# PN-CourseWork/02689-AdvancedNumericalAlgorithmP3

Hardware: AMD Instinct MI355X
Metric: steady-state time-steps/sec at N=256 Re=1000 (higher is better)
Workload: dtype f64; 1 GPU; solver=spectral (SG) N=256 Re=1000 fp64, full solve() iteration (dt, 4 RK stages + BCs, change/residual norms, E/Z/P), fluid from rest; N=256, trials_per_gpu=1, parallelism=1 independent trial(s), one per GPU

## Files before the change

02689-advancednumericalalgorithmp3_amd/csrc/ldc_kernels.hip:

```cpp

#include <hip/hip_runtime.h>
#include <stdint.h>
#include <stdlib.h>
#include <string.h>
#include <mutex>
#include <new>
#include <type_traits>
#include <vector>

#include "ldc_hip.h"

namespace {

typedef double v4d __attribute__((ext_vector_type(4)));

#define MFMA_F64(a, b, c) __builtin_amdgcn_mfma_f64_16x16x4f64((a), (b), (c), 0, 0, 0)

#ifdef LDC_TIMING
#define LDC_ABL(x, bits) ((x).ablate & (bits))
#else
#define LDC_ABL(x, bits) 0
#endif

constexpr int kWaves = 4;
// ... 175 lines not shown
  const int jj = loc / pr, i = loc - jj * pr;
  I = pI * pr + i;
  J = pJ * pc + (I + jj) % pc;
}

struct FinalArgs {
  int nblk4, nblkZ, nblkP;
  int with_diag, warmup, nan_guard, rec_cap;
  int do_critical;
  double cfl, beta2, nu, hx, hy, lid, tol;
  const double *part4, *partZ0, *partP0;
  long long stride;
  double* scal;
  int* ctrl;
  double* rec;
};

__device__ __forceinline__ double dt_lambda_x(double umax, const FinalArgs& a) {
  const double um = fmax(umax, a.lid);
  return (um + sqrt(nm_madd(um, um, a.beta2))) / a.hx + a.nu / (a.hx * a.hx);
}
__device__ __forceinline__ double dt_lambda_y(double vmax, const FinalArgs& a) {
  const double vm = fmax(vmax, 1e-10);
  return (vm + sqrt(nm_madd(vm, vm, a.beta2))) / a.hy + a.nu / (a.hy * a.hy);
}
__device__ __forceinline__ double next_dt(double umax, double vmax, const FinalArgs& a) {
  return a.cfl / (dt_lambda_x(umax, a) + dt_lambda_y(vmax, a));
}

struct TrialState {
  int done, iter, step, flushed, pdone, drows;
  int abort;
  unsigned arrive;
  double dt, umax, vmax;
  double dtp;
};

struct StageArgs {
  int M, LD, T, tail;
  int Mx, My;
  double nu, beta2, alpha;
  const double *Dx, *D2x, *Dy, *D2y, *IxF, *GxF;
  const double *Uin, *UinT, *Vin, *VinT;
  const double *U0, *V0, *P0;
  const double *U0T, *V0T;
  const double *T1T, *T2T;
  double *PX, *PY;
  double *Uout, *UoutT, *Vout, *VoutT, *Pout;
  const double *ulid, *wx, *wy;
  const double *DxL, *D2xL, *DyL, *D2yL;
  double *W, *WT;
  double *partZ0, *partP0;
  long long stride;
  const double* scal;
  int* ctrl;
  double* partials;
#ifdef LDC_TIMING
  int ablate;
#endif
  double* dump[11];
  int NB;
  const double *DxK, *D2xK, *DyK, *D2yK, *IxFK, *GxFK;
  const double *UinK, *UinTK, *VinK, *VinTK, *T1TK, *T2TK;
  double *UoutK, *UoutTK, *VoutK, *VoutTK, *PoutK, *WK, *WTK;
  int wt;
  int rm_out;
// ... 2340 lines not shown
```

02689-advancednumericalalgorithmp3_amd/csrc/ldc_wide_kernel.inc:

```

constexpr int kWT = 16;
constexpr int kWTmin = 6;
constexpr int kWD2 = 6;
constexpr int kWD = 4;

struct WArgs {
  int M, LD, NB, T;
  int tail;
  int Mx, My;
  int with_diag;
  double nu, beta2;
  const double *DxK, *D2xK, *DyK, *D2yK, *GxFK, *GyFK;
  const double *ulid, *wx, *wy;
  double *U, *UT, *V, *VT, *P;
  double *UK[3], *UTK[3], *VK[3], *VTK[3], *PK[3];
  double *PTK[3];
  double *WK, *WTK;
  const double *IxF, *IyF;
  const double *Dx, *D2x, *Dy, *D2y, *GxF, *GyF;
  const double *DxL, *D2xL, *DyL, *D2yL;
  double* wedge;
  double* jobs;
  double* ring;
  double* rvec;
// ... 54 lines not shown
  const v2d_t hi = *reinterpret_cast<const v2d_t*>(f + 128 + 2 * lane);
  return (v4d){lo[0], lo[1], hi[0], hi[1]};
}

__device__ __forceinline__ bool wwait_flags(unsigned* flags, unsigned phase, int T, int I, int J, bool all, int lane) {
  const int nwg = T * T;
  int wg[4] = {-1, -1, -1, -1};
  if (all) {
#pragma unroll
    for (int k = 0; k < 4; ++k) wg[k] = (lane + 64 * k < nwg) ? lane + 64 * k : -1;
  } else if (lane < 2 * T) {
    wg[0] = lane < T ? I * T + lane : (lane - T) * T + J;
  }
  unsigned long long t0 = 0;
  for (unsigned spins = 0;; ++spins) {
    unsigned v[4];
#pragma unroll
    for (int k = 0; k < 4; ++k)
      v[k] = ((k == 0 || all) && wg[k] >= 0) ? __hip_atomic_load((LDC_GLOBAL unsigned*)flags + 32 * wg[k], __ATOMIC_RELAXED, __HIP_MEMORY_SCOPE_AGENT) : phase;
    const bool behind = (v[0] < phase) || (v[1] < phase) || (v[2] < phase) || (v[3] < phase);
    if (__builtin_amdgcn_ballot_w64(behind) == 0ull) return true;
    if ((spins & 63u) == 63u) {
      const unsigned long long t = __builtin_amdgcn_s_memrealtime();
      if (t0 == 0) t0 = t;
      else if (t - t0 > kSpinLimitTicks) return false;
    }
  }
}
__device__ __forceinline__ void wgive_up(WArgsC& a, TrialState* S) {
  S->abort = 1;
  __hip_atomic_store((LDC_GLOBAL unsigned*)a.giveup, 1u, __ATOMIC_RELAXED, __HIP_MEMORY_SCOPE_AGENT);
}

__device__ __forceinline__ bool wbar(WArgsC& a, unsigned& phaseA, int T, int bx, int I, int J, int tid, TrialState* S, bool all,
                                     double* stp = nullptr) {
  asm volatile("s_waitcnt vmcnt(0)" ::: "memory");
  WSTAMP(7);
  __syncthreads();
  WSTAMP(8);
  ++phaseA;
  if (tid < 64) {
    if (tid == 0) __hip_atomic_store((LDC_GLOBAL unsigned*)a.flags + 32 * bx, phaseA, __ATOMIC_RELAXED, __HIP_MEMORY_SCOPE_AGENT);
    if (!wwait_flags(a.flags, phaseA, T, I, J, all, tid) && tid == 0) wgive_up(a, S);
    WSTAMP(9);
  }
  __syncthreads();
  WSTAMP(10);
  return S->abort == 0;
}

__device__ __forceinline__ v4d wld4(const double* base, size_t i) {
  const __amdgpu_buffer_rsrc_t r = raw_rsrc(base);
  const int off = (int)(i * sizeof(double));
  const v2d_t lo = __builtin_bit_cast(v2d_t, __builtin_amdgcn_raw_buffer_load_b128(r, off, 0, 16));
  const v2d_t hi = __builtin_bit_cast(v2d_t, __builtin_amdgcn_raw_buffer_load_b128(r, off + 16, 0, 16));
  return (v4d){lo[0], lo[1], hi[0], hi[1]};
}
__device__ __forceinline__ int wrows_padded(int nwg) { return (nwg + 3) & ~3; }

template <bool CONST_A>
__device__ __forceinline__ void wchain2(v4d& r0, v4d& r1, const double* p0, const double* p1, const double* pan, int NB,
                                        int prow, int T, int lane) {
  constexpr int D = kWD2;
  v4d f[D];
#pragma unroll
  for (int d = 0; d < D; ++d) {
    f[d] = ldpk_t<true>(pan, NB, prow, d, lane);
    __builtin_amdgcn_sched_barrier(0);
  }
  v4d c0[2], c1[2];
#pragma unroll
  for (int h = 0; h < 2; ++h) { c0[h] = (v4d){0.0, 0.0, 0.0, 0.0}; c1[h] = (v4d){0.0, 0.0, 0.0, 0.0}; }
  auto mm = [&](const v4d& x, int g) {
    const v4d k0 = wfrag_lds(p0 + g * 256, lane), k1 = wfrag_lds(p1 + g * 256, lane);
#pragma unroll
    for (int s = 0; s < 4; ++s) {
      if (CONST_A) { c0[s & 1] = MFMA_F64(k0[s], x[s], c0[s & 1]); c1[s & 1] = MFMA_F64(k1[s], x[s], c1[s & 1]); }
      else         { c0[s & 1] = MFMA_F64(x[s], k0[s], c0[s & 1]); c1[s & 1] = MFMA_F64(x[s], k1[s], c1[s & 1]); }
    }
  };
  int g = 0;
// ... 189 lines not shown
};
constexpr int kWJobDoubles = 16 * 16;
constexpr double kWJobTag = 7.25e22 + 1977.0;
enum { WJ_UE = 0, WJ_VE, WJ_CD0, WJ_CD1, WJ_CD2, WJ_CD3, WJ_PGS, WJ_PGR, WJ_OMEGA, WJ_WQ, WJ_OPL, WJ_CE0, WJ_CE1, WJ_CE2, WJ_CE3, WJ_UNI };
__device__ __forceinline__ int wjob_id(int kind, int blk, int T) { return kind == 0 ? blk : kind == 1 ? T + blk : 2 * T; }
__device__ __forceinline__ void wjob_load(WArgsC& a, WJob& jb, int T, int lane) {
  const double* base = a.jobs + (size_t)wjob_id(jb.kind, jb.blk, T) * kWJobDoubles;
  const int r = wopaque(lane) & 15;
  jb.ue = xld(base, WJ_UE * 16 + r); jb.ve = xld(base, WJ_VE * 16 + r);
  jb.cd[0] = xld(base, WJ_CD0 * 16 + r); jb.cd[1] = xld(base, WJ_CD1 * 16 + r);
  jb.cd[2] = xld(base, WJ_CD2 * 16 + r); jb.cd[3] = xld(base, WJ_CD3 * 16 + r);
  jb.ce[0] = xld(base, WJ_CE0 * 16 + r); jb.ce[1] = xld(base, WJ_CE1 * 16 + r);
  jb.ce[2] = xld(base, WJ_CE2 * 16 + r); jb.ce[3] = xld(base, WJ_CE3 * 16 + r);
  jb.pgs = xld(base, WJ_PGS * 16 + r); jb.pgr = xld(base, WJ_PGR * 16 + r);
  jb.omega = xld(base, WJ_OMEGA * 16 + r); jb.wq = xld(base, WJ_WQ * 16 + r); jb.opl = xld(base, WJ_OPL * 16 + r);
  jb.am1 = xld(base, WJ_UNI * 16 + 0); jb.am2 = xld(base, WJ_UNI * 16 + 1); jb.wc = xld(base, WJ_UNI * 16 + 2);
}
__device__ __forceinline__ void wjob_store(WArgsC& a, const WJob& jb, int T, int lane_, bool all) {
  const int lane = wopaque(lane_);
  double* base = a.jobs + (size_t)wjob_id(jb.kind, jb.blk, T) * kWJobDoubles;
  if (lane < 16) {
    wst1(base + WJ_PGS * 16 + lane, jb.pgs); wst1(base + WJ_PGR * 16 + lane, jb.pgr); wst1(base + WJ_OMEGA * 16 + lane, jb.omega);
    if (all) {
      wst1(base + WJ_UE * 16 + lane, jb.ue); wst1(base + WJ_VE * 16 + lane, jb.ve);
      wst1(base + WJ_CD0 * 16 + lane, jb.cd[0]); wst1(base + WJ_CD1 * 16 + lane, jb.cd[1]);
      wst1(base + WJ_CD2 * 16 + lane, jb.cd[2]); wst1(base + WJ_CD3 * 16 + lane, jb.cd[3]);
      wst1(base + WJ_CE0 * 16 + lane, jb.ce[0]); wst1(base + WJ_CE1 * 16 + lane, jb.ce[1]);
      wst1(base + WJ_CE2 * 16 + lane, jb.ce[2]); wst1(base + WJ_CE3 * 16 + lane, jb.ce[3]);
      wst1(base + WJ_WQ * 16 + lane, jb.wq); wst1(base + WJ_OPL * 16 + lane, jb.opl);
      if (lane == 0) { wst1(base + WJ_UNI * 16 + 0, jb.am1); wst1(base + WJ_UNI * 16 + 1, jb.am2); wst1(base + WJ_UNI * 16 + 2, jb.wc); }
    }
  }
}
enum { WR_JOBLINE = 64, WR_EXTRA = 96, WR_CGX = 97, WR_CGY = 98, WR_CPX = 99, WR_CPY = 100, WR_JOBRING2 = 104 };

struct WEdgeLoads { double ra[4], rb[4]; v4d f0[4], f1[4]; };
template <int MODE, bool DIAGV>
__device__ __forceinline__ void wedge_issue(WEdgeLoads& w, WArgsC& a, int kind, int blk, const XStageIo io, int T, int w4, int lane_) {
  const int lane = wopaque(lane_);
  const int NB = a.NB;
  const size_t rowm = (size_t)(a.M - 1) * a.LD;
  const double *pan0, *pan1, *rA, *rB;
  if (MODE == 1) {
    pan0 = kind == 0 ? a.VTK[io.in] : a.UK[io.in]; pan1 = kind == 0 ? a.PTK[io.pin] : a.PK[io.pin];
    rA = (kind == 0 ? a.Dx : a.Dy) + rowm; rB = (kind == 0 ? a.GxF : a.GyF) + rowm;
  } else if (MODE == 3) {
    pan0 = kind == 0 ? a.WTK : a.WK; pan1 = pan0;
    rA = (kind == 0 ? a.Dx : a.Dy) + rowm; rB = rA;
  } else {
    pan0 = kind == 0 ? a.UTK[io.in] : a.UK[io.in]; pan1 = kind == 0 ? a.VTK[io.in] : a.VK[io.in];
    rA = (kind == 0 ? a.Dx : a.Dy) + rowm; rB = (kind == 0 ? a.D2x : a.D2y) + rowm;
  }
  constexpr bool use0 = !(MODE == 1 && !DIAGV), use1 = MODE != 3;
#pragma unroll
  for (int m = 0; m < 4; ++m) {
    const int g = w4 + 4 * m, gc = g < T ? g : T - 1;
    const int ko = 16 * gc + 4 * (lane >> 4) + (lane & 3);
    w.ra[m] = *(const LDC_GLOBAL double*)(rA + ko);
    w.rb[m] = use1 ? *(const LDC_GLOBAL double*)(rB + ko) : w.ra[m];
    if (g >= T) { w.ra[m] = 0.0; w.rb[m] = 0.0; }
  }
#pragma unroll
  for (int m = 0; m < 4; ++m) {
    const int g = w4 + 4 * m, gc = g < T ? g : T - 1;
    w.f0[m] = use0 ? ldpk_t<true>(pan0, NB, blk, gc, lane) : (v4d){0.0, 0.0, 0.0, 0.0};
    w.f1[m] = use1 ? ldpk_t<true>(pan1, NB, blk, gc, lane) : w.f0[m];
// ... 151 lines not shown
    G[m] = ldpk(kind == 0 ? a.GxFK : a.GyFK, NB, kind == 0 ? I : J, g, lane);
  }
  for (int m0 = 0; m0 < nblk; m0 += 4) {
    const int m = m0 + (lane >> 4), r = lane & 15;
    const int B = half + 2 * (m < nblk ? m : 0);
    double t[kWT];
#pragma unroll
    for (int L = 0; L < kWT; ++L) {
      const int Lc = L < T ? L : T - 1;
      const size_t o = (size_t)(kind == 0 ? B * T + Lc : Lc * T + B) * 64 + (kind == 0 ? 0 : 32) + c * 16 + r;
      t[L] = xld(a.ring, o);
    }
    double s = 0.0;
#pragma unroll
    for (int L = 0; L < kWT; ++L) s += (L < T) ? t[L] : 0.0;
    if (m < nblk) vec[16 * B + r] = s;
  }
  asm volatile("s_waitcnt lgkmcnt(0)" ::: "memory");
  double s = 0.0;
#pragma unroll
  for (int m = 0; m < (kWT + 1) / 2; ++m) {
    if (m < nblk) {
      const int g = half + 2 * m;
      const v4d av = *reinterpret_cast<const v4d*>(vec + 16 * g + 4 * (lane >> 4));
      s = nm_madd(G[m][0], av[0], s); s = nm_madd(G[m][1], av[1], s);
      s = nm_madd(G[m][2], av[2], s); s = nm_madd(G[m][3], av[3], s);
    }
  }
  s = quad_sum(s);
  if (lane < 16) lds[Ld.RNG + (kind * 2 + half) * 16 + lane] = s;
}

struct WFoldState { bool crit, flush; double umax, vmax; };
__device__ __forceinline__ WFoldState wfold_dt(WArgsC& a, TrialState* S, int T, int I, int J, int lane, unsigned phaseA,
                                               v4d (&fx)[PS_N + 2], double* stp) {
  WFoldState f = {false, false, 0.0, 0.0};
  if (!wwait_flags(a.flags, phaseA, T, I, J, true, lane)) {
    if (lane == 0) wgive_up(a, S);
    return f;
  }
  WSTAMP(1);
  __builtin_amdgcn_s_setprio(3);
  FinalArgs fin;
  __builtin_memcpy(&fin, &a.fin, sizeof(FinalArgs));
  f.crit = fin.do_critical && !S->done && (S->step > S->iter);
  f.flush = fin.with_diag && (S->flushed < S->iter) && (S->pdone >= S->iter);
  const int nwg = T * T, nwp = wrows_padded(nwg), r0 = 4 * lane;
  const bool in = r0 < nwp;
#pragma unroll
  for (int q = 0; q < PS_N + 2; ++q) fx[q] = (v4d){0.0, 0.0, 0.0, 0.0};
  if (f.crit && in) {
    fx[PS_UMAX] = wld4(a.part4, (size_t)PS_UMAX * nwp + r0);
    fx[PS_VMAX] = wld4(a.part4, (size_t)PS_VMAX * nwp + r0);
#pragma unroll
    for (int q = 0; q < PS_NSUM; ++q) fx[q] = wld4(a.part4, (size_t)q * nwp + r0);
  }
  if (f.flush && in) {
    const size_t off = (size_t)((S->iter - 1) & 1) * a.stride + r0;
    fx[PS_N] = wld4(a.partZ0, off);
    fx[PS_N + 1] = wld4(a.partP0, off);
  }
  if (f.crit) {
    auto top = [&](const v4d& x) {
      const double e0 = (r0 < nwg) ? x[0] : 0.0, e1 = (r0 + 1 < nwg) ? x[1] : 0.0;
      const double e2 = (r0 + 2 < nwg) ? x[2] : 0.0, e3 = (r0 + 3 < nwg) ? x[3] : 0.0;
      return wave_top(fmax(fmax(e0, e1), fmax(e2, e3)));
    };
    f.umax = top(fx[PS_UMAX]); f.vmax = top(fx[PS_VMAX]);
  }
  WSTAMP(9);
  return f;
}
__device__ __forceinline__ void wfold_step(WArgsC& a, TrialState* S, const WFoldState& f, int lane) {
  if (f.crit) {
    FinalArgs fin;
    __builtin_memcpy(&fin, &a.fin, sizeof(FinalArgs));
    const double xr = lane == 0 ? dt_lambda_x(f.umax, fin) : lane == 1 ? dt_lambda_y(f.vmax, fin) : 0.0;
    const double lxy = lane_value(xr, 0) + lane_value(xr, 1);
    const double dt_new = fin.cfl / lxy;
    if (lane == 0) { S->dtp = S->dt; S->dt = dt_new; }
  }
  __builtin_amdgcn_s_setprio(0);
}
__device__ __forceinline__ void wfold_record(WArgsC& a, const WLds& Ld, double* lds, TrialState* S, int T, int lane, bool writer,
                                             const WFoldState f, const v4d (&fx)[PS_N + 2], double* stp) {
  if (!f.crit && !f.flush) return;
  FinalArgs fin;
  __builtin_memcpy(&fin, &a.fin, sizeof(FinalArgs));
  const int nwg = T * T, r0 = 4 * lane;
  double* tot = lds + Ld.TOT;
#pragma unroll
  for (int q = 0; q < PS_N + 2; ++q) {
    const double e0 = (r0 < nwg) ? fx[q][0] : 0.0, e1 = (r0 + 1 < nwg) ? fx[q][1] : 0.0;
    const double e2 = (r0 + 2 < nwg) ? fx[q][2] : 0.0, e3 = (r0 + 3 < nwg) ? fx[q][3] : 0.0;
    const bool is_max = (q == PS_UMAX || q == PS_VMAX);
    const double s = is_max ? fmax(fmax(e0, e1), fmax(e2, e3)) : ((e0 + e1) + (e2 + e3));
    const double t = is_max ? wave_top(s) : wave_total(s);
    if (lane == 0) tot[q] = t;
  }
  asm volatile("s_waitcnt lgkmcnt(0)" ::: "memory");
  WSTAMP(11);
  const double dt_cur = f.crit ? S->dtp : S->dt;
  const FinOut o = fin_decide_wave(fin, tot, lane, f.crit, f.flush, S->iter, S->flushed, dt_cur, writer);
  if (lane == 0) {
// ... 55 lines not shown
    const double* pan = wv == 0 ? a.UTK[io.in] : wv == 1 ? a.VTK[io.in] : wv == 2 ? a.UK[io.in] : a.VK[io.in];
    const double* p0 = ops + (xrole ? 0 : 2) * T * 256;
    v4d c0, c1;
    if (xrole) wchain2<true>(c0, c1, p0, p0 + T * 256, pan, NB, J, T, lane);
    else wchain2<false>(c0, c1, p0, p0 + T * 256, pan, NB, I, T, lane);
    WSTAMP(1);
    wput(lds, Ld, wv == 0 ? XR_UX : wv == 1 ? XR_VX : wv == 2 ? XR_UY : XR_VY, c0, lane);
    wput(lds, Ld, wv == 0 ? XR_UXX : wv == 1 ? XR_VXX : wv == 2 ? XR_UYY : XR_VYY, c1, lane);
  } else {
    if (PUBZ && wv == 7 && lane == 0) {
      const double* r = rsum;
      const double x = (((r[0] + r[1]) + (r[2] + r[3])) + ((r[4] + r[5]) + (r[6] + r[7]))) +
                       (((r[8] + r[9]) + (r[10] + r[11])) + ((r[12] + r[13]) + (r[14] + r[15])));
      const int step0 = S->step;
      wst1(a.partZ0 + (size_t)((step0 > 0 ? step0 - 1 : 0) & 1) * a.stride + wopaque_s(bx), TAIL ? x + r[16] : x);
    }
    if (GPV) {
      constexpr bool THREE = !(SP && K == 3);
      const int c1 = THREE ? (2 * T + 1) / 3 : T;
      if (wv == 4) wput(lds, Ld, XR_PX, wchain1<false, true>(nullptr, a.GxFK, I, a.PTK[io.pin], J, NB, c1, lane), lane);
      else if (wv == 5) wput(lds, Ld, XR_PY, wchain1<false, false>(nullptr, a.GyFK, J, a.PK[io.pin], I, NB, c1, lane), lane);
      else if (THREE && wv == 6) {
        wput(lds, Ld, XR_WX, wchain1<false, true>(nullptr, a.GxFK, I, a.PTK[io.pin], J, NB, T - c1, lane, c1), lane);
        wput(lds, Ld, XR_WY, wchain1<false, false>(nullptr, a.GyFK, J, a.PK[io.pin], I, NB, T - c1, lane, c1), lane);
      }
    }
    if (AGRADW) {
      const int h0 = (T + 1) / 2, g0 = wv < 6 ? 0 : h0, ng = wv < 6 ? h0 : T - h0;
      if ((wv & 1) == 0) wput(lds, Ld, wv == 4 ? XR_PX : XR_WX, wchain1<true, true>(ops, nullptr, 0, a.WTK, J, NB, ng, lane, g0), lane);
      else wput(lds, Ld, wv == 5 ? XR_PY : XR_WY, wchain1<true, false>(ops + 2 * T * 256, nullptr, 0, a.WK, I, NB, ng, lane, g0), lane);
    }
    if (RRED && wv == 7 && I == J) wring_reduce(a, T, I, lane);
    if (K == 0 && wv == 7 && fold) {
      fs = wfold_dt(a, S, T, I, J, lane, phaseA, fx, stp);
      wfold_step(a, S, fs, lane);
    }
    if (TAIL && LAST && job) {
      const size_t rowm = (size_t)(a.M - 1) * a.LD;
      const int q0 = (wv - 4) * T / 4, q1 = (wv - 3) * T / 4;
      if (DIAGV && jb.kind < 2) wvec_issue(jvh, a.wedge, jb.kind == 0 ? 0 : (size_t)16 * kWT, q0, q1 - q0, lane);
      if (wv >= 6) wjob_load(a, jb, T, lane);
      if (jb.kind < 2) wedge_issue<4, DIAGV>(jw, a, jb.kind, jb.blk, io, T, wv - 4, lane);
      if (DIAGV && jb.kind == 2 && wv == 7) {
        const double* jbase = a.jobs + (size_t)wjob_id(2, 0, T) * kWJobDoubles;
        const int l4 = 4 * wopaque(lane), n4 = 16 * T;
        jw.ra[0] = xld(jbase, WJ_UNI * 16 + 0); jw.ra[1] = xld(jbase, WJ_UNI * 16 + 1); jw.ra[2] = xld(jbase, WJ_UNI * 16 + 2);
        const bool in = l4 < n4;
        const int lc = in ? l4 : 0;
        jw.f0[0] = *(const LDC_GLOBAL v4d*)(a.Dx + rowm + lc); jw.f0[1] = wld4(a.wedge, (size_t)16 * kWT + lc);
        jw.f0[2] = *(const LDC_GLOBAL v4d*)(a.Dy + rowm + lc); jw.f0[3] = wld4(a.wedge, (size_t)lc);
        if (!in) { jw.f0[0] = (v4d){0.0, 0.0, 0.0, 0.0}; jw.f0[2] = jw.f0[0]; }
      }
      WSTAMP(1);
    }
    if (TAIL && K == 1 && wv == 6 && job) wjob_load(a, jb, T, lane);
    if (RING3 && wv >= 6) {
      if (!wwait_flags(a.flags, phaseA, T, I, J, true, lane)) {
        if (lane == 0) wgive_up(a, S);
      } else {
        if (J == 0 || J == jLast) wring(a, Ld, lds, T, I, J, lane, wv - 6, 0, J == 0 ? 0 : 1);
        if (I == 0 || I == iLast) wring(a, Ld, lds, T, I, J, lane, wv - 6, 1, I == 0 ? 0 : 1);
      }
    }
  }
  WSTAMP(2);
  __syncthreads();
  WSTAMP(3);
  if (S->abort != 0) return false;
  double v[PS_N], ev[PS_N];
#pragma unroll
  for (int q = 0; q < PS_N; ++q) ev[q] = 0.0;
  if (TAIL && K == 1 && wv == 6 && job) { wedge_finish<1, DIAGV>(a, Ld, lds, jb, lane, ev); wjob_store(a, jb, T, lane, false); }
  if (TAIL && LAST && job && wv >= 4) {
    if (jb.kind < 2) wedge_dots<4, DIAGV>(jw, Ld, lds, wv - 4, lane);
    if (DIAGV && jb.kind < 2) {
      const int q0 = (wv - 4) * T / 4, q1 = (wv - 3) * T / 4;
      wvec_finish(jvh, jb.kind == 0 ? ops + 2 * T * 256 : ops, nullptr, 0, NB, q0, q1 - q0, lane, lds + Ld.AXY + 320 + 16 * (wv - 4));
    }
    if (DIAGV && jb.kind == 2 && wv == 7) {
      double sx = 0.0, sy = 0.0;
#pragma unroll
      for (int e = 0; e < 4; ++e) { sx = nm_madd(jw.f0[0][e], jw.f0[1][e], sx); sy = nm_madd(jw.f0[2][e], jw.f0[3][e], sy); }
      const double gxc = wave_total(sx) + jw.ra[0] * jw.ra[2], gyc = wave_total(sy) + jw.ra[1] * jw.ra[2];
      if (lane == 0) { rng[WR_CGX] = gxc; rng[WR_CGY] = gyc; }
    }
  }
  if (tid < 256) {
    auto C = [&](int slot) { return lds[Ld.RES + (slot * 4 + wv) * 64 + lane]; };
    double ux = C(XR_UX), vx = C(XR_VX), uy = C(XR_UY), vy = C(XR_VY);
    double lu = C(XR_UXX) + C(XR_UYY), lv = C(XR_VXX) + C(XR_VYY);
    if (TAIL) { ux += tn.cux; vx += tn.cvx; uy += tn.cuy; vy += tn.cvy; lu += tn.clu; lv += tn.clv; }
    const int blkIJ = I * NB + J, blkJI = J * NB + I;
    double dsum = 0.0;
    if (GPV) {
      constexpr bool THREE = !(SP && K == 3);
      n.px = n.valid ? (THREE ? C(XR_PX) + C(XR_WX) : C(XR_PX)) : 0.0;
      n.py = n.valid ? (THREE ? C(XR_PY) + C(XR_WY) : C(XR_PY)) : 0.0;
    }
    if (RINGE) {
      if (n.rc >= 0) n.px = rng[n.ti];
      if (n.rr >= 0) n.py = rng[32 + n.tj];
    }
    if (RING3) {
      if (n.rc >= 0) n.px = rng[n.ti] + rng[16 + n.ti];
      if (n.rr >= 0) n.py = rng[32 + n.tj] + rng[48 + n.tj];
    }
    if (DIAGE == 1) {
      const double w = n.valid ? (vx - uy) : 0.0;
      wst(a.WK, blkIJ, n.oU, w);
      wst(a.WTK, blkJI, n.oT, w);
      dsum = n.valid ? n.wq * w * w : 0.0;
    }
    if (DIAGE == 2) {
      double gx = C(XR_PX) + C(XR_WX), gy = C(XR_PY) + C(XR_WY);
      if (TAIL) { gx = nm_madd(tn.dxl, wre, gx); gy = nm_madd(wce, tn.dyl, gy); }
      dsum = n.valid ? n.wq * nm_sq2(gx, gy) : 0.0;
    }
    const double Ru = nm_momentum(n.uc, n.vc, ux, uy, n.px, a.nu, lu);
// ... 6 lines not shown
    else if (n.wall) { un = 0.0; vn = 0.0; }
    wst(a.UK[io.out], blkIJ, n.oU, un);
    wst(a.UTK[io.out], blkJI, n.oT, un);
    wst(a.VK[io.out], blkIJ, n.oU, vn);
    wst(a.VTK[io.out], blkJI, n.oT, vn);
    double pn = 0.0;
    if (has_p) {
      pn = n.interior ? nm_madd(adt, Rp, n.p0) : 0.0;
      wst(a.PK[io.pout], blkIJ, n.oU, pn);
      wst(a.PTK[io.pout], blkJI, n.oT, pn);
      if (RPROD) wring_partials(a, Ld, n, lds, pn, bx, lane, wv);
    }
    if (LAST) {
      const double du = un - n.u0, dv = vn - n.v0;
      v[PS_DU2] = n.valid ? du * du : 0.0;
      v[PS_DV2] = n.valid ? dv * dv : 0.0;
      v[PS_U02] = n.valid ? n.u0 * n.u0 : 0.0;
      v[PS_V02] = n.valid ? n.v0 * n.v0 : 0.0;
      v[PS_RU2] = n.valid ? Ru * Ru : 0.0;
      v[PS_RV2] = n.valid ? Rv * Rv : 0.0;
      v[PS_RP2] = n.interior ? Rp * Rp : 0.0;
      v[PS_E] = n.valid ? n.wq * nm_sq2(un, vn) : 0.0;
      v[PS_UMAX] = fabs(un);
      v[PS_VMAX] = fabs(vn);
      n.u0 = un; n.v0 = vn; n.p0 = pn;
    }
    if (DIAGE != 0) {
      const double r = row16_sum(dsum);
      if ((lane & 15) == 0) rsum[n.ti] = r;
    }
    n.uc = un; n.vc = vn;
  }
  WSTAMP(4);
  if (LAST || RPROD) {
    __syncthreads();
    WSTAMP(5);
    if (RPROD) wring_partials_finish(a, Ld, lds, bx, tid);
    if (LAST) {
      constexpr int RS = TAIL ? 272 : 256;
      double* red = lds + Ld.RES;
      if (tid < 256) {
#pragma unroll
        for (int q = 0; q < PS_N; ++q) red[q * RS + tid] = v[q];
      }
      if (TAIL && wv == 7 && job) wedge_finish<5, DIAGV>(a, Ld, lds, jb, lane, ev);
      if (TAIL && wv == 6) {
        if (job) { wedge_finish<3, DIAGV>(a, Ld, lds, jb, lane, ev); wedge_finish<4, DIAGV>(a, Ld, lds, jb, lane, ev); }
        if (lane < 16) {
#pragma unroll
          for (int q = 0; q < PS_N; ++q) red[q * RS + 256 + lane] = ev[q];
        }
      }
      __syncthreads();
      const int nwp = wrows_padded(nwg);
      {
        const double* r = red + wv * RS + lane;
        double y = ((r[0] + r[64]) + r[128]) + r[192];
        if (TAIL) y += (lane < 16) ? r[256] : 0.0;
        const double x = wave_sum(y);
        if (lane == 0) wst1(a.part4 + (size_t)wv * nwp + wopaque_s(bx), x);
      }
      if (wv < 2) {
        const double* r = red + (PS_NSUM + wv) * RS + lane;
        double y = fmax(fmax(r[0], r[64]), fmax(r[128], r[192]));
        if (TAIL) y = fmax(y, (lane < 16) ? r[256] : 0.0);
        const double x = wave_max(y);
        if (lane == 0) wst1(a.part4 + (size_t)(PS_NSUM + wv) * nwp + wopaque_s(bx), x);
      }
      if (DIAGV && tid == 64 * 3) {
        const double* r = rsum;
        const double x = (((r[0] + r[1]) + (r[2] + r[3])) + ((r[4] + r[5]) + (r[6] + r[7]))) +
                         (((r[8] + r[9]) + (r[10] + r[11])) + ((r[12] + r[13]) + (r[14] + r[15])));
        const int step0 = S->step;
        wst1(a.partP0 + (size_t)((step0 > 0 ? step0 - 1 : 0) & 1) * a.stride + wopaque_s(bx), TAIL ? x + r[16] : x);
        S->pdone = step0; S->drows = nwg;
      }
      if (tid == 0) S->step = S->step + 1;
    }
  }
  WSTAMP(6);
  asm volatile("s_waitcnt vmcnt(0)" ::: "memory");
  WSTAMP(7);
  ++phaseA;
  if (lane == 0) __hip_atomic_fetch_add(&S->arrive, 1u, __ATOMIC_RELAXED, __HIP_MEMORY_SCOPE_WORKGROUP);
  if (wv == 0) {
    const unsigned want = 8u * (phaseA - 1u);
    while (__hip_atomic_load(&S->arrive, __ATOMIC_RELAXED, __HIP_MEMORY_SCOPE_WORKGROUP) < want) __builtin_amdgcn_s_sleep(1);
    WSTAMP(8);
    if (tid == 0) __hip_atomic_store((LDC_GLOBAL unsigned*)a.flags + 32 * bx, phaseA, __ATOMIC_RELAXED, __HIP_MEMORY_SCOPE_AGENT);
    if (!wwait_flags(a.flags, phaseA, T, I, J, false, tid) && tid == 0) wgive_up(a, S);
    WSTAMP(9);
  } else if (wv >= 4) {
    if (K == 0 && wv == 7 && fold) wfold_record(a, Ld, lds, S, T, lane, bx == 0, fs, fx, stp);
    if (TAIL && K == 0 && job && jb.kind < 2 && wv < 7) {
      wedge_stream<1, DIAGV>(a, Ld, lds, jb.kind, jb.blk, io, T, wv - 4, lane);
      if (wv == 6) wedge_stream<1, DIAGV>(a, Ld, lds, jb.kind, jb.blk, io, T, 3, lane);
    }
    if (WLINES) {
      if (wv == 4 && (J == 0 || J == jLast)) wring_line(a, T, I, lane, 0, J == 0 ? 0 : 1, rng);
      if (wv == 5 && (I == 0 || I == iLast)) wring_line(a, T, J, lane, 1, I == 0 ? 0 : 1, rng + 32);
      if (job) {
        const size_t rowm = (size_t)(a.M - 1) * a.LD;
        if (DIAGV && jb.kind < 2) wedge_stream<3, DIAGV>(a, Ld, lds, jb.kind, jb.blk, io, T, wv - 4, lane);
        if (wv >= 6 && jb.kind < 2) {
          const int h0 = (T + 1) / 2, g0 = wv == 6 ? 0 : h0, ng = wv == 6 ? h0 : T - h0;
          const int lk = jb.kind == 0 ? 1 : 0;
          WVecHalf vh;
          wvec_issue(vh, a.rvec, (size_t)(2 * lk + 1) * 16 * T, g0, ng, lane);
          wvec_finish(vh, nullptr, lk == 0 ? a.GxFK : a.GyFK, jb.blk, NB, g0, ng, lane,
                      wv == 6 ? rng + (jb.kind == 0 ? 48 : 16) : rng + WR_JOBRING2);
          if (wv == 7 && jb.blk == 0) {
            const double e = jb.kind == 0 ? wvv(a.GxF + rowm, a.rvec, 0, 16 * T, lane)
                                          : wvv(a.GyF + rowm, a.rvec, (size_t)2 * 16 * T, 16 * T, lane);
            if (lane == 0) rng[WR_EXTRA] = e;
          }
        } else if (wv == 6 && jb.kind == 2) {
          const double pxc = wvv(a.GxF + rowm, a.rvec, (size_t)16 * T, 16 * T, lane);
          const double pyc = wvv(a.GyF + rowm, a.rvec, (size_t)3 * 16 * T, 16 * T, lane);
          if (lane == 0) { rng[WR_CPX] = pxc; rng[WR_CPY] = pyc; }
        }
      }
    }
  }
  __syncthreads();
  WSTAMP(10);
  return S->abort == 0;
}

template <bool SP, bool DIAGV, bool TAIL>
__global__ __launch_bounds__(kStageThreads, 2) void wide_kernel(const WLaunch L) {
  static_assert(!(SP && DIAGV), "the smoother carries no diagnostics");
  static_assert(!(SP && TAIL), "the tail layout is built for SG");
  extern __shared__ __attribute__((aligned(16))) double lds[];
  __shared__ TrialState S;
  const int tid = threadIdx.x, lane = tid & 63;
  const int wv = __builtin_amdgcn_readfirstlane(tid >> 6);
  WArgsC& a0 = L.trials ? *(WArgsC*)(uintptr_t)L.trials
                        : *(WArgsC*)((kernarg_ptr)__builtin_amdgcn_kernarg_segment_ptr() + __builtin_offsetof(WLaunch, one));
  const int T = a0.T, nwg = T * T;
  const int trial = (int)blockIdx.x / nwg, bx = (int)blockIdx.x % nwg;
  WArgsC& a = L.trials ? *(WArgsC*)(uintptr_t)(L.trials + trial) : a0;
  const WLds Ld = wlds_of(T);
  const int NB = a.NB, M = a.M, LD = a.LD;
  const int I = bx / T, J = bx % T;
  if (a.fin.ctrl[LDC_CTRL_DONE] != 0) return;
  if (tid == 0) {
    S.done = a.fin.ctrl[LDC_CTRL_DONE]; S.iter = a.fin.ctrl[LDC_CTRL_ITER]; S.step = a.fin.ctrl[LDC_CTRL_STEP];
    S.flushed = a.fin.ctrl[LDC_CTRL_FLUSHED]; S.pdone = a.fin.ctrl[LDC_CTRL_PDONE]; S.drows = a.fin.ctrl[LDC_CTRL_DROWS];
    S.dt = a.fin.scal[LDC_SCAL_DT]; S.umax = a.fin.scal[LDC_SCAL_UMAX]; S.vmax = a.fin.scal[LDC_SCAL_VMAX];
    S.abort = 0; S.arrive = 0u; S.dtp = 0.0;
  }
  for (int q = tid; q < 4 * T * 256; q += kStageThreads) {
    const int p = q / (T * 256), r = q - p * (T * 256), g = r >> 8, e = r & 255;
    const double* src = p == 0 ? a.DxK : p == 1 ? a.D2xK : p == 2 ? a.DyK : a.D2yK;
    const int row = p < 2 ? I : J;
    lds[Ld.OPS + (p * T + g) * 256 + ((e & 3) >> 1) * 128 + (e >> 2) * 2 + (e & 1)] = src[((size_t)(row * NB + g) << 8) + e];
  }
  XNode n;
  n.ti = 4 * (wv & 3) + (lane >> 4); n.tj = lane & 15;
  n.i = 16 * I + n.ti; n.j = 16 * J + n.tj;
  n.oU = xpk(n.ti, n.tj); n.oT = xpk(n.tj, n.ti);
  const int Mx = a.Mx, My = a.My;
  n.valid = (n.i < Mx) && (n.j < My);
  n.interior = (n.i >= 1) && (n.i <= Mx - 2) && (n.j >= 1) && (n.j <= My - 2);
  n.lid = n.valid && (n.j == My - 1);
  n.wall = n.valid && (n.i == 0 || n.i == Mx - 1 || n.j == 0);
  n.rc = !n.valid ? -1 : n.j == 0 ? 0 : n.j == My - 1 ? 1 : -1;
  n.rr = !n.valid ? -1 : n.i == 0 ? 0 : n.i == Mx - 1 ? 1 : -1;
  n.u0 = n.v0 = n.p0 = n.px = n.py = n.lidv = n.wq = 0.0;
  const size_t ij = (size_t)n.i * LD + n.j;
  if (tid < 64) {
    const int c = (tid >> 4) & 1, e = tid & 15;
    const size_t row = c ? (size_t)((tid < 32 ? My : Mx) - 1) * LD : 0;
    lds[Ld.EYX + tid] = (tid < 32) ? a.IyF[row + 16 * J + e] : a.IxF[row + 16 * I + e];
  }
  if (tid < 256) {
    n.u0 = a.U[ij]; n.v0 = a.V[ij]; n.p0 = a.P[ij];
    n.lidv = a.ulid[n.i];
    n.wq = a.wx[n.i] * a.wy[n.j];
    wst(a.UK[0], I * NB + J, n.oU, n.u0); wst(a.UTK[0], J * NB + I, n.oT, n.u0);
    wst(a.VK[0], I * NB + J, n.oU, n.v0); wst(a.VTK[0], J * NB + I, n.oT, n.v0);
    wst(a.PK[0], I * NB + J, n.oU, n.p0);
    wst(a.PTK[0], J * NB + I, n.oT, n.p0);
// ... 25 lines not shown
        WJob jb;
        wjob_init(a, jb, T, I, J, lane);
        wjob_store(a, jb, T, lane, true);
        if (lane == 0) wst1(jbase + WJ_UNI * 16 + 3, kWJobTag);
      }
    }
    if (tid < 16) lds[Ld.RSUM + 16 + tid] = 0.0;
  }
  unsigned phaseA = 0;
  bool alive = wbar(a, phaseA, T, bx, I, J, tid, &S, true);
  bool pending = false;
  for (int it = 0; alive && it < L.n_iters; ++it) {
    if (S.done != 0) break;
#ifdef LDC_TIMING
    const bool stamp = a.stamps != nullptr && it == L.n_iters - 1;
#else
    const bool stamp = false;
#endif
    alive = wstage<SP, DIAGV, TAIL, 0>(a, Ld, n, tn, jkind, jblk, lds, &S, phaseA, T, bx, I, J, pending, stamp);
    if (!alive) break;
    pending = false;
    if (S.done != 0) break;
    alive = wstage<SP, DIAGV, TAIL, 1>(a, Ld, n, tn, jkind, jblk, lds, &S, phaseA, T, bx, I, J, false, stamp);
    if (!alive) break;
    alive = wstage<SP, DIAGV, TAIL, 2>(a, Ld, n, tn, jkind, jblk, lds, &S, phaseA, T, bx, I, J, false, stamp);
    if (!alive) break;
    alive = wstage<SP, DIAGV, TAIL, 3>(a, Ld, n, tn, jkind, jblk, lds, &S, phaseA, T, bx, I, J, false, stamp);
    pending = true;
  }
  if (!alive) return;
  if (pending) {
    if (wv == 7) {
      v4d fx[PS_N + 2];
      const WFoldState fs = wfold_dt(a, &S, T, I, J, lane, phaseA, fx, nullptr);
      wfold_step(a, &S, fs, lane);
      wfold_record(a, Ld, lds, &S, T, lane, bx == 0, fs, fx, nullptr);
    }
    __syncthreads();
    if (S.abort != 0) return;
  }
  double* tu = lds + Ld.RES;
  double* tv = tu + 16 * 17;
  if (tid < 256) {
    a.U[ij] = n.u0; a.V[ij] = n.v0; a.P[ij] = n.p0;
    tu[n.ti * 17 + n.tj] = n.u0; tv[n.ti * 17 + n.tj] = n.v0;
  }
  __syncthreads();
  if (tid < 256) {
    const int tr = tid >> 4, tc = tid & 15;
    const size_t ot = (size_t)(16 * J + tr) * LD + 16 * I + tc;
    a.UT[ot] = tu[tc * 17 + tr];
    a.VT[ot] = tv[tc * 17 + tr];
  }
  if (bx == 0 && tid == 0) {
    a.fin.ctrl[LDC_CTRL_DONE] = S.done; a.fin.ctrl[LDC_CTRL_ITER] = S.iter; a.fin.ctrl[LDC_CTRL_STEP] = S.step;
    a.fin.ctrl[LDC_CTRL_FLUSHED] = S.flushed; a.fin.ctrl[LDC_CTRL_PDONE] = S.pdone; a.fin.ctrl[LDC_CTRL_DROWS] = S.drows;
    a.fin.ctrl[LDC_CTRL_LIVE] = 0;
    a.fin.scal[LDC_SCAL_DT] = S.dt; a.fin.scal[LDC_SCAL_UMAX] = S.umax; a.fin.scal[LDC_SCAL_VMAX] = S.vmax;
  }
}
```

Baseline: 28370 steps/s.

## Publish per-block velocity maxima in flag words to shorten dt critical path

Each workgroup now publishes its u/v maxima, tagged with parity sign bits, directly in its flag cache line. The dt fold can then read all maxima from the flags without waiting for the full partial-sum reduction. The final stage's workgroup barrier is split into per-wave arrive counters (P, D, E, S), so the maxima publish and inter-block flag release happen before the ten partial-sum reductions finish. A separate sums flag gates the later partial loads. This shortens the serial dt dependency between RK iterations, at the cost of more intricate sync logic, extra counters and possible ordering bugs.

```diff
diff --git a/02689-advancednumericalalgorithmp3_amd/csrc/ldc_kernels.hip b/02689-advancednumericalalgorithmp3_amd/csrc/ldc_kernels.hip
--- a/02689-advancednumericalalgorithmp3_amd/csrc/ldc_kernels.hip
+++ b/02689-advancednumericalalgorithmp3_amd/csrc/ldc_kernels.hip
@@ -231,6 +231,7 @@
   int done, iter, step, flushed, pdone, drows;
   int abort;
   unsigned arrive;
+  unsigned arriveP, arriveD, arriveE, arriveS;
   double dt, umax, vmax;
   double dtp;
 };
diff --git a/02689-advancednumericalalgorithmp3_amd/csrc/ldc_wide_kernel.inc b/02689-advancednumericalalgorithmp3_amd/csrc/ldc_wide_kernel.inc
--- a/02689-advancednumericalalgorithmp3_amd/csrc/ldc_wide_kernel.inc
+++ b/02689-advancednumericalalgorithmp3_amd/csrc/ldc_wide_kernel.inc
@@ -110,6 +110,71 @@
   __hip_atomic_store((LDC_GLOBAL unsigned*)a.giveup, 1u, __ATOMIC_RELAXED, __HIP_MEMORY_SCOPE_AGENT);
 }
 
+constexpr int kWFlagSums = 2;
+constexpr int kWFlagMaxBytes = 16;
+constexpr unsigned long long kWSignBit = 1ull << 63;
+__host__ __device__ inline unsigned long long wmax_encode(double x, unsigned sign) {
+  return (__builtin_bit_cast(unsigned long long, x) & ~kWSignBit) | (sign ? kWSignBit : 0ull);
+}
+__host__ __device__ inline double wmax_decode(unsigned long long w) { return __builtin_bit_cast(double, w & ~kWSignBit); }
+__host__ __device__ inline bool wmax_pair_valid(unsigned long long u, unsigned long long v, unsigned parity) {
+  return (unsigned)(u >> 63) == (parity & 1u) && (unsigned)(v >> 63) == ((parity & 1u) ^ 1u);
+}
+__device__ __forceinline__ unsigned witers_of(unsigned phaseA) { return (phaseA - 1u) >> 2; }
+
+__device__ __forceinline__ void wpublish_maxima(unsigned* flags, int bx, double umax, double vmax, unsigned parity) {
+  LDC_GLOBAL unsigned long long* w = (LDC_GLOBAL unsigned long long*)(flags + 32 * bx) + kWFlagMaxBytes / 8;
+  __hip_atomic_store(w, wmax_encode(umax, parity & 1u), __ATOMIC_RELAXED, __HIP_MEMORY_SCOPE_AGENT);
+  __hip_atomic_store(w + 1, wmax_encode(vmax, (parity & 1u) ^ 1u), __ATOMIC_RELAXED, __HIP_MEMORY_SCOPE_AGENT);
+}
+__device__ __forceinline__ bool wwait_maxima(unsigned* flags, unsigned parity, int nwg, int lane, double& umax, double& vmax) {
+  const __amdgpu_buffer_rsrc_t rs = raw_rsrc((const double*)flags);
+  const int r0 = 4 * lane;
+  unsigned long long t0 = 0;
+  for (unsigned spins = 0;; ++spins) {
+    double u[4], v[4];
+    bool behind = false;
+    asm volatile("" ::: "memory");
+#pragma unroll
+    for (int k = 0; k < 4; ++k) {
+      u[k] = 0.0; v[k] = 0.0;
+      if (r0 + k < nwg) {
+        typedef unsigned long long v2u64 __attribute__((ext_vector_type(2)));
+        const v2u64 w = __builtin_bit_cast(v2u64, __builtin_amdgcn_raw_buffer_load_b128(rs, 128 * (r0 + k) + kWFlagMaxBytes, 0, 16));
+        behind = behind || !wmax_pair_valid(w[0], w[1], parity);
+        u[k] = wmax_decode(w[0]); v[k] = wmax_decode(w[1]);
+      }
+    }
+    if (__builtin_amdgcn_ballot_w64(behind) == 0ull) {
+      umax = fmax(fmax(u[0], u[1]), fmax(u[2], u[3]));
+      vmax = fmax(fmax(v[0], v[1]), fmax(v[2], v[3]));
+      return true;
+    }
+    if ((spins & 63u) == 63u) {
+      const unsigned long long t = __builtin_amdgcn_s_memrealtime();
+      if (t0 == 0) t0 = t;
+      else if (t - t0 > kSpinLimitTicks) return false;
+    }
+  }
+}
+__device__ __forceinline__ bool wwait_sums(unsigned* flags, unsigned count, int nwg, int lane) {
+  const int r0 = 4 * lane;
+  unsigned long long t0 = 0;
+  for (unsigned spins = 0;; ++spins) {
+    bool behind = false;
+#pragma unroll
+    for (int k = 0; k < 4; ++k)
+      if (r0 + k < nwg)
+        behind = behind || __hip_atomic_load((LDC_GLOBAL unsigned*)flags + 32 * (r0 + k) + kWFlagSums, __ATOMIC_RELAXED, __HIP_MEMORY_SCOPE_AGENT) < count;
+    if (__builtin_amdgcn_ballot_w64(behind) == 0ull) return true;
+    if ((spins & 63u) == 63u) {
+      const unsigned long long t = __builtin_amdgcn_s_memrealtime();
+      if (t0 == 0) t0 = t;
+      else if (t - t0 > kSpinLimitTicks) return false;
+    }
+  }
+}
+
 __device__ __forceinline__ bool wbar(WArgsC& a, unsigned& phaseA, int T, int bx, int I, int J, int tid, TrialState* S, bool all,
                                      double* stp = nullptr) {
   asm volatile("s_waitcnt vmcnt(0)" ::: "memory");
@@ -125,6 +190,15 @@
   __syncthreads();
   WSTAMP(10);
   return S->abort == 0;
+}
+
+__device__ __forceinline__ void warrive(unsigned* c, int lane) {
+  asm volatile("s_waitcnt lgkmcnt(0)" ::: "memory");
+  if (lane == 0) __hip_atomic_fetch_add(c, 1u, __ATOMIC_RELAXED, __HIP_MEMORY_SCOPE_WORKGROUP);
+}
+__device__ __forceinline__ void wawait(unsigned* c, unsigned want) {
+  while (__hip_atomic_load(c, __ATOMIC_RELAXED, __HIP_MEMORY_SCOPE_WORKGROUP) < want) __builtin_amdgcn_s_sleep(1);
+  asm volatile("" ::: "memory");
 }
 
 __device__ __forceinline__ v4d wld4(const double* base, size_t i) {
@@ -380,6 +454,7 @@
     }
   }
 }
+enum { WRS_JOBSUM = 16, WRS_WAVEMAX = 20, WRS_JOBMAX = 28 };
 enum { WR_JOBLINE = 64, WR_EXTRA = 96, WR_CGX = 97, WR_CGY = 98, WR_CPX = 99, WR_CPY = 100, WR_JOBRING2 = 104 };
 
 struct WEdgeLoads { double ra[4], rb[4]; v4d f0[4], f1[4]; };
@@ -597,23 +672,39 @@
 }
 
 struct WFoldState { bool crit, flush; double umax, vmax; };
-__device__ __forceinline__ WFoldState wfold_dt(WArgsC& a, TrialState* S, int T, int I, int J, int lane, unsigned phaseA,
-                                               v4d (&fx)[PS_N + 2], double* stp) {
+__device__ __forceinline__ WFoldState wfold_dt(WArgsC& a, TrialState* S, int T, int lane, unsigned phaseA, double* stp) {
   WFoldState f = {false, false, 0.0, 0.0};
-  if (!wwait_flags(a.flags, phaseA, T, I, J, true, lane)) {
-    if (lane == 0) wgive_up(a, S);
-    return f;
-  }
-  WSTAMP(1);
-  __builtin_amdgcn_s_setprio(3);
   FinalArgs fin;
   __builtin_memcpy(&fin, &a.fin, sizeof(FinalArgs));
   f.crit = fin.do_critical && !S->done && (S->step > S->iter);
   f.flush = fin.with_diag && (S->flushed < S->iter) && (S->pdone >= S->iter);
+  __builtin_amdgcn_s_setprio(3);
+  if (f.crit) {
+    double um = 0.0, vm = 0.0;
+    if (!wwait_maxima(a.flags, witers_of(phaseA), T * T, lane, um, vm)) {
+      if (lane == 0) wgive_up(a, S);
+      f.crit = false; f.flush = false;
+      return f;
+    }
+    WSTAMP(1);
+    f.umax = wave_top(um); f.vmax = wave_top(vm);
+  }
+  WSTAMP(9);
+  return f;
+}
+__device__ __forceinline__ void wfold_loads(WArgsC& a, TrialState* S, WFoldState& f, int T, int lane, unsigned phaseA,
+                                            v4d (&fx)[PS_N + 2], double* stp) {
   const int nwg = T * T, nwp = wrows_padded(nwg), r0 = 4 * lane;
   const bool in = r0 < nwp;
 #pragma unroll
   for (int q = 0; q < PS_N + 2; ++q) fx[q] = (v4d){0.0, 0.0, 0.0, 0.0};
+  if (!f.crit && !f.flush) return;
+  if (!wwait_sums(a.flags, witers_of(phaseA), nwg, lane)) {
+    if (lane == 0) wgive_up(a, S);
+    f.crit = false; f.flush = false;
+    return;
+  }
+  WSTAMP(5);
   if (f.crit && in) {
     fx[PS_UMAX] = wld4(a.part4, (size_t)PS_UMAX * nwp + r0);
     fx[PS_VMAX] = wld4(a.part4, (size_t)PS_VMAX * nwp + r0);
@@ -625,16 +716,6 @@
     fx[PS_N] = wld4(a.partZ0, off);
     fx[PS_N + 1] = wld4(a.partP0, off);
   }
-  if (f.crit) {
-    auto top = [&](const v4d& x) {
-      const double e0 = (r0 < nwg) ? x[0] : 0.0, e1 = (r0 + 1 < nwg) ? x[1] : 0.0;
-      const double e2 = (r0 + 2 < nwg) ? x[2] : 0.0, e3 = (r0 + 3 < nwg) ? x[3] : 0.0;
-      return wave_top(fmax(fmax(e0, e1), fmax(e2, e3)));
-    };
-    f.umax = top(fx[PS_UMAX]); f.vmax = top(fx[PS_VMAX]);
-  }
-  WSTAMP(9);
-  return f;
 }
 __device__ __forceinline__ void wfold_step(WArgsC& a, TrialState* S, const WFoldState& f, int lane) {
   if (f.crit) {
@@ -756,8 +837,9 @@
     }
     if (RRED && wv == 7 && I == J) wring_reduce(a, T, I, lane);
     if (K == 0 && wv == 7 && fold) {
-      fs = wfold_dt(a, S, T, I, J, lane, phaseA, fx, stp);
+      fs = wfold_dt(a, S, T, lane, phaseA, stp);
       wfold_step(a, S, fs, lane);
+      wfold_loads(a, S, fs, T, lane, phaseA, fx, stp);
     }
     if (TAIL && LAST && job) {
       const size_t rowm = (size_t)(a.M - 1) * a.LD;
@@ -795,19 +877,10 @@
 #pragma unroll
   for (int q = 0; q < PS_N; ++q) ev[q] = 0.0;
   if (TAIL && K == 1 && wv == 6 && job) { wedge_finish<1, DIAGV>(a, Ld, lds, jb, lane, ev); wjob_store(a, jb, T, lane, false); }
-  if (TAIL && LAST && job && wv >= 4) {
-    if (jb.kind < 2) wedge_dots<4, DIAGV>(jw, Ld, lds, wv - 4, lane);
-    if (DIAGV && jb.kind < 2) {
-      const int q0 = (wv - 4) * T / 4, q1 = (wv - 3) * T / 4;
-      wvec_finish(jvh, jb.kind == 0 ? ops + 2 * T * 256 : ops, nullptr, 0, NB, q0, q1 - q0, lane, lds + Ld.AXY + 320 + 16 * (wv - 4));
-    }
-    if (DIAGV && jb.kind == 2 && wv == 7) {
-      double sx = 0.0, sy = 0.0;
-#pragma unroll
-      for (int e = 0; e < 4; ++e) { sx = nm_madd(jw.f0[0][e], jw.f0[1][e], sx); sy = nm_madd(jw.f0[2][e], jw.f0[3][e], sy); }
-      const double gxc = wave_total(sx) + jw.ra[0] * jw.ra[2], gyc = wave_total(sy) + jw.ra[1] * jw.ra[2];
-      if (lane == 0) { rng[WR_CGX] = gxc; rng[WR_CGY] = gyc; }
-    }
+  if (TAIL && LAST && job && wv == 6) {
+    const bool own = jb.kind == 2 ? (lane == 0) : (lane < 16);
+    const double ju = wave_max(own ? fabs(jb.ue) : 0.0), jv = wave_max(own ? fabs(jb.ve) : 0.0);
+    if (lane == 0) { rsum[WRS_JOBMAX] = ju; rsum[WRS_JOBMAX + 1] = jv; }
   }
   if (tid < 256) {
     auto C = [&](int slot) { return lds[Ld.RES + (slot * 4 + wv) * 64 + lane]; };
@@ -880,51 +953,112 @@
     n.uc = un; n.vc = vn;
   }
   WSTAMP(4);
-  if (LAST || RPROD) {
+  if (LAST) {
     __syncthreads();
     WSTAMP(5);
-    if (RPROD) wring_partials_finish(a, Ld, lds, bx, tid);
-    if (LAST) {
-      constexpr int RS = TAIL ? 272 : 256;
-      double* red = lds + Ld.RES;
-      if (tid < 256) {
-#pragma unroll
-        for (int q = 0; q < PS_N; ++q) red[q * RS + tid] = v[q];
-      }
-      if (TAIL && wv == 7 && job) wedge_finish<5, DIAGV>(a, Ld, lds, jb, lane, ev);
-      if (TAIL && wv == 6) {
-        if (job) { wedge_finish<3, DIAGV>(a, Ld, lds, jb, lane, ev); wedge_finish<4, DIAGV>(a, Ld, lds, jb, lane, ev); }
-        if (lane < 16) {
+    ++phaseA;
+    const unsigned cnt = witers_of(phaseA);
+    constexpr int RS = TAIL ? 272 : 256;
+    double* red = lds + Ld.RES;
+    if (wv < 4) {
+      if (RPROD) wring_partials_finish(a, Ld, lds, bx, tid);
+#pragma unroll
+      for (int q = 0; q < PS_N; ++q) red[q * RS + tid] = v[q];
+      const double mu = wave_max(v[PS_UMAX]), mv = wave_max(v[PS_VMAX]);
+      if (lane == 0) { rsum[WRS_WAVEMAX + 2 * wv] = mu; rsum[WRS_WAVEMAX + 2 * wv + 1] = mv; }
+      asm volatile("s_waitcnt vmcnt(0)" ::: "memory");
+      WSTAMP(7);
+      warrive(&S->arriveP, lane);
+    }
+    if (wv == 0) {
+      wawait(&S->arriveP, 4u * cnt);
+      WSTAMP(8);
+      if (tid == 0) {
+        const double* m = rsum + WRS_WAVEMAX;
+        double mu = fmax(fmax(m[0], m[2]), fmax(m[4], m[6])), mv = fmax(fmax(m[1], m[3]), fmax(m[5], m[7]));
+        if (TAIL) { mu = fmax(mu, rsum[WRS_JOBMAX]); mv = fmax(mv, rsum[WRS_JOBMAX + 1]); }
+        wpublish_maxima(a.flags, bx, mu, mv, cnt);
+        __hip_atomic_store((LDC_GLOBAL unsigned*)a.flags + 32 * bx, phaseA, __ATOMIC_RELAXED, __HIP_MEMORY_SCOPE_AGENT);
+      }
+      if (!wwait_flags(a.flags, phaseA, T, I, J, false, tid) && tid == 0) wgive_up(a, S);
+      WSTAMP(9);
+    } else {
+      if (TAIL && wv >= 4) {
+        if (job) {
+          if (jb.kind < 2) wedge_dots<4, DIAGV>(jw, Ld, lds, wv - 4, lane);
+          if (DIAGV && jb.kind < 2) {
+            const int q0 = (wv - 4) * T / 4, q1 = (wv - 3) * T / 4;
+            wvec_finish(jvh, jb.kind == 0 ? ops + 2 * T * 256 : ops, nullptr, 0, NB, q0, q1 - q0, lane, lds + Ld.AXY + 320 + 16 * (wv - 4));
+          }
+          if (DIAGV && jb.kind == 2 && wv == 7) {
+            double sx = 0.0, sy = 0.0;
+#pragma unroll
+            for (int e = 0; e < 4; ++e) { sx = nm_madd(jw.f0[0][e], jw.f0[1][e], sx); sy = nm_madd(jw.f0[2][e], jw.f0[3][e], sy); }
+            const double gxc = wave_total(sx) + jw.ra[0] * jw.ra[2], gyc = wave_total(sy) + jw.ra[1] * jw.ra[2];
+            if (lane == 0) { rng[WR_CGX] = gxc; rng[WR_CGY] = gyc; }
+          }
+          warrive(&S->arriveD, lane);
+          if (wv >= 6) {
+            wawait(&S->arriveD, 4u * cnt);
+            if (wv == 7) wedge_finish<5, DIAGV>(a, Ld, lds, jb, lane, ev);
+            else { wedge_finish<3, DIAGV>(a, Ld, lds, jb, lane, ev); wedge_finish<4, DIAGV>(a, Ld, lds, jb, lane, ev); }
+          }
+        }
+        if (wv == 6 && lane < 16) {
 #pragma unroll
           for (int q = 0; q < PS_N; ++q) red[q * RS + 256 + lane] = ev[q];
         }
-      }
-      __syncthreads();
+        if (wv >= 6) warrive(&S->arriveE, lane);
+      }
+      wawait(&S->arriveP, 4u * cnt);
+      if (TAIL) wawait(&S->arriveE, 2u * cnt);
       const int nwp = wrows_padded(nwg);
-      {
-        const double* r = red + wv * RS + lane;
-        double y = ((r[0] + r[64]) + r[128]) + r[192];
-        if (TAIL) y += (lane < 16) ? r[256] : 0.0;
-        const double x = wave_sum(y);
-        if (lane == 0) wst1(a.part4 + (size_t)wv * nwp + wopaque_s(bx), x);
-      }
-      if (wv < 2) {
-        const double* r = red + (PS_NSUM + wv) * RS + lane;
-        double y = fmax(fmax(r[0], r[64]), fmax(r[128], r[192]));
-        if (TAIL) y = fmax(y, (lane < 16) ? r[256] : 0.0);
-        const double x = wave_max(y);
-        if (lane == 0) wst1(a.part4 + (size_t)(PS_NSUM + wv) * nwp + wopaque_s(bx), x);
-      }
-      if (DIAGV && tid == 64 * 3) {
-        const double* r = rsum;
-        const double x = (((r[0] + r[1]) + (r[2] + r[3])) + ((r[4] + r[5]) + (r[6] + r[7]))) +
-                         (((r[8] + r[9]) + (r[10] + r[11])) + ((r[12] + r[13]) + (r[14] + r[15])));
+      auto reduce = [&](int q) {
+        const double* r = red + q * RS + lane;
+        double x;
+        if (q < PS_NSUM) {
+          double y = ((r[0] + r[64]) + r[128]) + r[192];
+          if (TAIL) y += (lane < 16) ? r[256] : 0.0;
+          x = wave_sum(y);
+        } else {
+          double y = fmax(fmax(r[0], r[64]), fmax(r[128], r[192]));
+          if (TAIL) y = fmax(y, (lane < 16) ? r[256] : 0.0);
+          x = wave_max(y);
+        }
+        if (lane == 0) wst1(a.part4 + (size_t)q * nwp + wopaque_s(bx), x);
+      };
+      static_assert(PS_N == 10 && kStageWaves == 8, "ten values over the waves 1-7");
+      if (wv < 4) { reduce(wv - 1); reduce(wv + 2); }
+      else reduce(wv + 2);
+      if (wv == 7 && lane == 0) {
         const int step0 = S->step;
-        wst1(a.partP0 + (size_t)((step0 > 0 ? step0 - 1 : 0) & 1) * a.stride + wopaque_s(bx), TAIL ? x + r[16] : x);
-        S->pdone = step0; S->drows = nwg;
-      }
-      if (tid == 0) S->step = S->step + 1;
-    }
+        if (DIAGV) {
+          const double* r = rsum;
+          const double x = (((r[0] + r[1]) + (r[2] + r[3])) + ((r[4] + r[5]) + (r[6] + r[7]))) +
+                           (((r[8] + r[9]) + (r[10] + r[11])) + ((r[12] + r[13]) + (r[14] + r[15])));
+          wst1(a.partP0 + (size_t)((step0 > 0 ? step0 - 1 : 0) & 1) * a.stride + wopaque_s(bx), TAIL ? x + r[16] : x);
+          S->pdone = step0; S->drows = nwg;
+        }
+        S->step = step0 + 1;
+      }
+      WSTAMP(6);
+      asm volatile("s_waitcnt vmcnt(0)" ::: "memory");
+      WSTAMP(7);
+      warrive(&S->arriveS, lane);
+      if (wv == 7) {
+        wawait(&S->arriveS, 7u * cnt);
+        if (lane == 0) __hip_atomic_store((LDC_GLOBAL unsigned*)a.flags + 32 * bx + kWFlagSums, cnt, __ATOMIC_RELAXED, __HIP_MEMORY_SCOPE_AGENT);
+        WSTAMP(8);
+      }
+    }
+    __syncthreads();
+    WSTAMP(10);
+    return S->abort == 0;
+  }
+  if (RPROD) {
+    __syncthreads();
+    WSTAMP(5);
+    wring_partials_finish(a, Ld, lds, bx, tid);
   }
   WSTAMP(6);
   asm volatile("s_waitcnt vmcnt(0)" ::: "memory");
@@ -932,7 +1066,7 @@
   ++phaseA;
   if (lane == 0) __hip_atomic_fetch_add(&S->arrive, 1u, __ATOMIC_RELAXED, __HIP_MEMORY_SCOPE_WORKGROUP);
   if (wv == 0) {
-    const unsigned want = 8u * (phaseA - 1u);
+    const unsigned want = 8u * (phaseA - 1u - witers_of(phaseA));
     while (__hip_atomic_load(&S->arrive, __ATOMIC_RELAXED, __HIP_MEMORY_SCOPE_WORKGROUP) < want) __builtin_amdgcn_s_sleep(1);
     WSTAMP(8);
     if (tid == 0) __hip_atomic_store((LDC_GLOBAL unsigned*)a.flags + 32 * bx, phaseA, __ATOMIC_RELAXED, __HIP_MEMORY_SCOPE_AGENT);
@@ -997,6 +1131,7 @@
     S.flushed = a.fin.ctrl[LDC_CTRL_FLUSHED]; S.pdone = a.fin.ctrl[LDC_CTRL_PDONE]; S.drows = a.fin.ctrl[LDC_CTRL_DROWS];
     S.dt = a.fin.scal[LDC_SCAL_DT]; S.umax = a.fin.scal[LDC_SCAL_UMAX]; S.vmax = a.fin.scal[LDC_SCAL_VMAX];
     S.abort = 0; S.arrive = 0u; S.dtp = 0.0;
+    S.arriveP = 0u; S.arriveD = 0u; S.arriveE = 0u; S.arriveS = 0u;
   }
   for (int q = tid; q < 4 * T * 256; q += kStageThreads) {
     const int p = q / (T * 256), r = q - p * (T * 256), g = r >> 8, e = r & 255;
@@ -1088,8 +1223,9 @@
   if (pending) {
     if (wv == 7) {
       v4d fx[PS_N + 2];
-      const WFoldState fs = wfold_dt(a, &S, T, I, J, lane, phaseA, fx, nullptr);
+      WFoldState fs = wfold_dt(a, &S, T, lane, phaseA, nullptr);
       wfold_step(a, &S, fs, lane);
+      wfold_loads(a, &S, fs, T, lane, phaseA, fx, nullptr);
       wfold_record(a, Ld, lds, &S, T, lane, bx == 0, fs, fx, nullptr);
     }
     __syncthreads();
```

Measured after the change: 27060 steps/s. 0.954x the previous value.
